# trvon/yams

Measured on AMD Instinct MI355X. Metric: k-NN QPS + recall@k, 100M x 768 fp32 cosine top-100; ingest GB/s SHA-256+CDC, higher is better.
Workload: dtype i8 (MFMA filter, exact i32 accumulate) + f64 (exact re-score)

## Files before the change

yams_amd/csrc/scan_api.cpp:

```cpp
#include <chrono>
#include <algorithm>
#include <cmath>
#include <cstdio>
#include <cstdlib>
#include <cstring>
#include <vector>

#include "accel_ctx.h"
#include "scan_launch.h"

using namespace yams_accel;

namespace {

constexpr uint64_t kMfmaMinRows = 4096;
constexpr uint64_t kExactKeyBudget = 1ull << 31;
constexpr size_t kStatWords = 16;

uint32_t round_up(uint32_t v, uint32_t m) { return (v + m - 1) / m * m; }

ScanPlan make_plan(uint64_t n_rows, uint32_t dim, uint32_t nq, uint32_t k, bool bf16, int passes, bool l2_band, int depth = 0) {
    ScanPlan p;
    p.n_rows = n_rows; p.dim = dim; p.n_queries = nq;
    p.tile_rows = bf16 ? 256 : kTileRows;
// ... 460 lines not shown
    const uint32_t nq = b.nq; const bool i8 = f.i8, bf16 = f.bf16;
    ScanLaunch& L = f.L; const ScanPlan& plan = L.plan;
    if (i8) L.dense = nullptr;
    else YA_TRY(ws_get(ctx, "dense", static_cast<size_t>(nq) * plan.sample_rows * 4, (void**)&L.dense));
    YA_TRY(ws_get(ctx, "gmax", static_cast<size_t>(nq) * plan.n_groups * 4, (void**)&L.gmax));
    YA_TRY(ws_get(ctx, "tau", static_cast<size_t>(nq) * 4, (void**)&f.d_tau));
    YA_TRY(ws_get(ctx, "list", static_cast<size_t>(nq) * plan.list_cap * 8, (void**)&f.d_list));
    const uint32_t gchunks = (plan.n_groups + kSelectCap - 1) / kSelectCap;
    YA_TRY(ws_get(ctx, "work32", static_cast<size_t>(2) * nq * std::max(1u, gchunks) * plan.tau_rank * 4, (void**)&f.d_work32));
    const uint32_t lchunks = (plan.list_cap + kSelectCap - 1) / kSelectCap, keep_max = kRescoreMax + 1;
    YA_TRY(ws_get(ctx, "work64", static_cast<size_t>(2) * nq * lchunks * keep_max * 8, (void**)&f.d_work64));
    L.tau = f.d_tau; L.tau_out = f.d_tau; L.list_count = b.d_lcount; L.list = f.d_list;
    if (i8) {
        L.i8_q_form = i8_takes_q_form(L, f.bf16_version);
        if (corpus->row_mask && corpus->row_mask_count) L.i8_mask_inflation = static_cast<double>(corpus->n_rows) / static_cast<double>(corpus->row_mask_count);
        const uint64_t regions = i8_log_regions(L);
        L.log_cap = i8_log_capacity(L);
        YA_TRY(ws_get(ctx, "i8_log_key", static_cast<size_t>(regions) * L.log_cap * i8_log_entry_bytes(L), (void**)&L.log_key));
        YA_TRY(ws_get(ctx, "i8_log_q", static_cast<size_t>(regions) * L.log_cap * 4, (void**)&L.log_q));
        const uint64_t sync_words = i8_sync_words(L);
        const size_t z_cnt = (static_cast<size_t>(regions) * 4 + 255) & ~size_t(255), z_over = (static_cast<size_t>(nq) * 4 + 255) & ~size_t(255);
        unsigned char* zeroed;
        YA_TRY(ws_get(ctx, "i8_zeroed", z_cnt + z_over + static_cast<size_t>(sync_words) * 4, (void**)&zeroed));
        YA_HIP(ctx, launch_prep_i8(st, b.d_qprep, nq, L.q_pad, b.dim, const_cast<int8_t*>(L.q_i8), const_cast<float*>(L.q_meta), L.i8_l2,
                                   reinterpret_cast<uint32_t*>(zeroed), (z_cnt + z_over) / 4 + sync_words, (corpus->i8_flags & YAMS_SCAN_I8_ROTATED) != 0));
        L.log_cnt = reinterpret_cast<uint32_t*>(zeroed);
        L.q_over = f.d_qover = reinterpret_cast<uint32_t*>(zeroed + z_cnt);
        if (sync_words) L.i8_sync = reinterpret_cast<uint32_t*>(zeroed + z_cnt + z_over);
    }
    { TimedRegion tr(ctx, "scan_sample");
      if (i8) YA_HIP(ctx, launch_scan_i8(st, L, 0, f.bf16_version));
      else if (bf16) YA_HIP(ctx, launch_scan_bf16(st, L, b.metric, 0, f.passes, f.bf16_version)); else YA_HIP(ctx, launch_scan_sample(st, L, b.metric));
      tr.end(); }
    if (b.retry) YA_HIP(ctx, hipMemcpyAsync(f.d_tau, b.retry->forced_tau, static_cast<size_t>(nq) * 4, hipMemcpyDeviceToDevice, st));
    else YA_HIP(ctx, launch_select_tau(st, L, f.d_work32));
    if (i8 && L.i8_l2) {
        YA_HIP(ctx, launch_i8_l2_thresholds(st, f.d_tau, L.q_meta, nq, L.q_pad, b.dim, b.d_l2_stats, const_cast<float*>(L.q_thr), const_cast<uint32_t*>(L.i8_q_bias)));
        YA_HIP(ctx, launch_i8_l2_rows(st, corpus->rows_nsq, corpus->rows_i8_meta, b.d_l2_nmin, corpus->n_rows, b.d_l2_stats, const_cast<float*>(L.i8_l2_meta),
                                      const_cast<uint8_t*>(L.i8_row_bias)));
    } else if (i8) YA_HIP(ctx, launch_i8_thresholds(st, f.d_tau, L.q_meta, nq, L.q_pad, const_cast<float*>(L.q_thr)));
    if (i8) YA_HIP(ctx, launch_i8_collect_sample(st, L)); else YA_HIP(ctx, launch_collect_sample(st, L));
    if (i8 && L.i8_l2) YA_HIP(ctx, launch_i8_l2_add_special(st, L, b.d_l2_special, b.l2_n_special));
    { GatedSweep gs(ctx, st);
      TimedRegion tr(ctx, "scan_filter");
      if (i8) YA_HIP(ctx, launch_scan_i8(st, L, 1, f.bf16_version));
      else if (bf16) YA_HIP(ctx, launch_scan_bf16(st, L, b.metric, 1, f.passes, f.bf16_version)); else YA_HIP(ctx, launch_scan_filter(st, L, b.metric));
      tr.end();
      gs.leave(); }
    if (i8) YA_HIP(ctx, launch_i8_log_gather(st, L));
#ifdef YAMS_ACCEL_MEASURE
    if (i8 && L.i8_sync) if (const char* dump = std::getenv("YAMS_ACCEL_DUMP_SYNC")) {
        std::vector<uint32_t> h(i8_sync_words(L));
        YA_HIP(ctx, hipMemcpyAsync(h.data(), L.i8_sync, h.size() * 4, hipMemcpyDeviceToHost, st));
        YA_HIP(ctx, hipStreamSynchronize(st));
        if (FILE* fp = std::fopen(dump, "wb")) { std::fwrite(h.data(), 4, h.size(), fp); std::fclose(fp); }
    }
    const int bv = f.bf16_version;
    if (bv != 2 && bv != 3 && bv != 4 && bv != 20 && bv != 30 && bv != 40 && bv != 50 && bv != 70 && bv != 80 && !(bv >= 81 && bv <= 99)) {
        YA_HIP(ctx, hipStreamSynchronize(st));
        YA_HIP(ctx, hipMemsetAsync(b.io.out_counts, 0, static_cast<size_t>(nq) * 4, st));
        *done = true;
    }
#endif
    return YAMS_OK;
}

yams_status_t rescore(const Batch& b, const Filter& f, uint32_t n_slots, const uint32_t* d_qmap, uint32_t n_cand) {
    const yams_scan_corpus_t* corpus = b.io.corpus;
    const uint64_t* res; uint64_t res_stride;
    YA_HIP(b.ctx, launch_select_lists(b.st, f.d_list, b.d_lcount, f.L.plan.list_cap, n_slots, d_qmap, n_cand + 1, f.d_work64, &res, &res_stride));
    RescoreLaunch R{};
    R.rows = corpus->rows; R.n_rows = corpus->n_rows; R.dim = b.dim; R.queries = b.io.queries; R.qnorm = b.d_qnorm; R.tie_rank = corpus->tie_rank;
    R.rank_row = nullptr; R.row_base = corpus->row_base; R.stripe_rows = corpus->stripe_rows; R.n_stripes = corpus->n_stripes;
    R.stripe_index = corpus->stripe_index; R.cand = res; R.cand_stride = res_stride; R.n_cand = n_cand; R.tau = f.d_tau; R.list_count = b.d_lcount;
// ... 431 lines not shown
```

yams_amd/csrc/scan_i8_kernel.hip:

```cpp
#include <cstdlib>
#include <type_traits>

#include "lds_dma.h"
#include "scan_args.h"

namespace yams_accel {

using i32x4v = __attribute__((ext_vector_type(4))) int;

constexpr int I8_ROWS = 256, I8_QUERIES = 256, I8_THREADS = 512;
constexpr int I8_SLAB = 64;
constexpr int I8_NST = 4;
constexpr int I8_A_BYTES = I8_ROWS * I8_SLAB;
constexpr int I8_B_BYTES = I8_QUERIES * I8_SLAB;
constexpr int I8_STAGE = I8_A_BYTES + I8_B_BYTES;
constexpr int I8_BLOCK_ROWS = 64;

__device__ __forceinline__ int i8_swz(int row) {
    const int j = (row >> 2) & 3;
    return (((j ^ (j >> 1)) & 1) << 1) | (j >> 1);
}

__host__ __device__ __forceinline__ uint64_t i8_blocked_offset(uint64_t row, uint32_t col, uint32_t dim) {
    const uint32_t j = static_cast<uint32_t>(row & 15u), slab = col >> 6, chunk = (col >> 4) & 3u;
    const uint32_t g = (j >> 2) & 3u, swz = (((g ^ (g >> 1)) & 1u) << 1) | (g >> 1);
    return ((row >> 4) * (dim >> 6) + slab) * 1024u + j * 64u + ((chunk ^ swz) << 4) + (col & 15u);
}

__device__ __forceinline__ int i8_neg_threshold(float A, float is, float B, float g) {
    const float t = fmaf(-A, is, fmaf(B, g, 2.0f));
    return static_cast<int>(__builtin_amdgcn_fmed3f(t, -1.0737418e9f, 1.0737418e9f));
}

__device__ __forceinline__ float i8_l2_bound(float u, float nsq, float eps) {
    const float t1 = sqrtf(nsq) * u;
    return fmaf(eps, fmaf(0.5f, nsq, fabsf(t1)), fmaf(-0.5f, nsq, t1));
}
// ... 875 lines not shown
    const uint32_t n = log_cnt[r];
    if (n == 0) return;
    const uint32_t q0 = ((r >> 3) % n_qt) * R_QUERIES;
    const int tid = threadIdx.x;
    if (tid < R_QUERIES) hist[tid] = 0u;
    __syncthreads();
    const uint64_t* keys = log_key + static_cast<uint64_t>(r) * log_cap;
    const uint32_t* qs = log_q + static_cast<uint64_t>(r) * log_cap;
    for (uint32_t i = tid; i < n; i += 256) {
        const uint32_t q = qs[i];
        uint32_t row; float u;
        if (!L2 || i8_entry_score<L2>(keys[i], q, rows_meta, q_meta, q_thr, l2, row, u)) atomicAdd(&hist[q - q0], 1u);
    }
    __syncthreads();
    if (tid < R_QUERIES) {
        const uint32_t c = hist[tid];
        slot0[tid] = c ? atomicAdd(&list_count[q0 + tid], c) : 0u;
        hist[tid] = 0u;
    }
    __syncthreads();
    for (uint32_t i = tid; i < n; i += 256) {
        const uint32_t q = qs[i];
        uint32_t row; float u;
        if (!i8_entry_score<L2>(keys[i], q, rows_meta, q_meta, q_thr, l2, row, u)) continue;
        const uint32_t pos = slot0[q - q0] + atomicAdd(&hist[q - q0], 1u);
        if (pos < list_cap) list[static_cast<uint64_t>(q) * list_cap + pos] = pack_key(u, row);
    }
}

#ifdef YAMS_ACCEL_MEASURE
#include "scan_i8q_gather.h"
#endif

__global__ __launch_bounds__(256) void i8_collect_sample_kernel(const uint32_t* gmax, uint32_t n_groups, uint32_t n_queries,
                                                                const int8_t* rows_i8, const float* rows_meta, const int8_t* q_i8,
                                                                const float* q_meta, uint32_t q_pad, uint32_t dim,
                                                                uint32_t stride, uint64_t n_rows, const uint32_t* row_mask,
                                                                const float* tau, uint32_t* list_count, uint64_t* list,
                                                                uint32_t list_cap, const float* l2_rows_nsq, float l2_eps) {
    const uint32_t q = blockIdx.y;
    const float t = tau[q];
    const uint32_t* gm = gmax + static_cast<uint64_t>(q) * n_groups;
    const uint32_t nchunk = dim / 16;
    const int lane = threadIdx.x & 63;
    const float4 qm = reinterpret_cast<const float4*>(q_meta)[q];
    const uint32_t wave0 = (blockIdx.x * blockDim.x + threadIdx.x) & ~63u, wstep = gridDim.x * blockDim.x;
    for (uint32_t g0 = wave0; g0 < n_groups; g0 += wstep) {
        const uint32_t gl = g0 + static_cast<uint32_t>(lane);
        const bool hot = gl < n_groups && !(ord2f(gm[gl]) < t);
        for (uint64_t hm = __builtin_amdgcn_ballot_w64(hot); hm; hm &= hm - 1) {
            const uint32_t g = g0 + static_cast<uint32_t>(__builtin_ctzll(hm));
            const int i = lane & 15;
            const uint64_t sidx = static_cast<uint64_t>(g >> 2) * 64 + 4 * (g & 3) + 16 * (i >> 2) + (i & 3);
            const uint64_t row = (sidx / I8_ROWS) * stride * I8_ROWS + (sidx % I8_ROWS);
            const bool ok = row < n_rows && (!row_mask || row_allowed(row_mask, row));
            const uint64_t rr = row < n_rows ? row : n_rows - 1;
            int dot = 0;
            for (uint32_t ch = static_cast<uint32_t>(lane >> 4); ch < nchunk; ch += 4) {
                const int4 xv = *reinterpret_cast<const int4*>(rows_i8 + i8_blocked_offset(rr, ch * 16, dim));
                const int4 qv = *reinterpret_cast<const int4*>(q_i8 + (static_cast<uint64_t>(ch >> 2) * q_pad + q) * 64 + (ch & 3u) * 16);
                dot = __builtin_amdgcn_sdot4(xv.x, qv.x, dot, false);
                dot = __builtin_amdgcn_sdot4(xv.y, qv.y, dot, false);
                dot = __builtin_amdgcn_sdot4(xv.z, qv.z, dot, false);
                dot = __builtin_amdgcn_sdot4(xv.w, qv.w, dot, false);
            }
            dot += __shfl_xor(dot, 16);
            dot += __shfl_xor(dot, 32);
            if (lane < 16 && ok) {
                const float2 bm = reinterpret_cast<const float2*>(rows_meta)[row / I8_BLOCK_ROWS];
                const float S = bm.x * qm.x, K = fmaf(bm.y, qm.y, qm.z);
                float u = fmaf(static_cast<float>(dot), S, K);
                bool unbounded = false;
                if (l2_rows_nsq) {
                    const float nsq = l2_rows_nsq[row];
                    unbounded = !norm_in_range(nsq);
                    u = i8_l2_bound(u, nsq, l2_eps);
                }
                if (!unbounded && !(u < t)) {
                    const uint32_t pos = atomicAdd(&list_count[q], 1u);
                    if (pos < list_cap) list[static_cast<uint64_t>(q) * list_cap + pos] = pack_key(u, static_cast<uint32_t>(row));
                }
            }
        }
    }
}

__device__ inline uint32_t rot_sign(uint32_t i, uint32_t salt) {
    uint32_t v = i * 2654435761u + salt * 0x9E3779B9u;
    v ^= v >> 15; v *= 2246822519u; v ^= v >> 13; v *= 3266489917u; v ^= v >> 16;
    return v << 31;
}
__device__ inline void wave_lds_fence() {
    __builtin_amdgcn_fence(__ATOMIC_ACQ_REL, "wavefront");
    __builtin_amdgcn_wave_barrier();
}
template <int EPL>
__device__ inline void wave_fwht(float* w, int lane, uint32_t g0, uint32_t sign_salt, float scale) {
    float v[EPL];
#pragma unroll
    for (int i = 0; i < EPL; ++i) {
        const uint32_t idx = static_cast<uint32_t>(lane) * EPL + i;
        float x = w[idx];
        if (sign_salt) x = __uint_as_float(__float_as_uint(x) ^ rot_sign(g0 + idx, sign_salt));
        v[i] = x;
    }
#pragma unroll
    for (int len = 1; len < EPL; len <<= 1)
#pragma unroll
        for (int i = 0; i < EPL; ++i)
            if (!(i & len)) { const float a = v[i], b = v[i + len]; v[i] = a + b; v[i + len] = a - b; }
#pragma unroll
    for (int m = 1; m < 64; m <<= 1)
#pragma unroll
        for (int i = 0; i < EPL; ++i) {
            const float o = __shfl_xor(v[i], m);
            v[i] = (lane & m) ? o - v[i] : v[i] + o;
// ... 527 lines not shown
#ifdef YAMS_ACCEL_MEASURE
bool i8_takes_q_form(const ScanLaunch& L, int version) {
    if (L.i8_l2 || L.plan.dim % (64u * Q_DEPTH) != 0 || L.plan.dim < 128u * Q_DEPTH) return false;
    if (!i8_resident_plan(L).use) return false;
    return version >= 70 && version <= 72;
}
uint32_t i8_log_entry_bytes(const ScanLaunch& L) { return L.i8_q_form ? Q_BLK_DWORDS * 4u : 8u; }
#else
bool i8_takes_q_form(const ScanLaunch&, int) { return false; }
uint32_t i8_log_entry_bytes(const ScanLaunch&) { return 8u; }
#endif

uint64_t i8_log_regions(const ScanLaunch& L) {
    const ResidentPlan r = i8_resident_plan(L);
    if (r.use && L.i8_q_form) return static_cast<uint64_t>(r.n_streams) * r.n_qt * 4u;
    if (r.use) return static_cast<uint64_t>(r.n_streams) * r.n_qt * 8u;
    return static_cast<uint64_t>((2u * L.plan.n_filter_tiles + 7) / 8) * L.plan.n_qtiles * 8u * 4u;
}

hipError_t launch_i8_collect_sample(hipStream_t st, const ScanLaunch& L) {
    if (L.plan.sample_rows == 0 || L.plan.n_groups == 0) return hipSuccess;
    uint32_t gx = (L.plan.n_groups + 255) / 256;
    if (gx > 64) gx = 64;
#ifdef YAMS_ACCEL_MEASURE
    if (const char* e = std::getenv("YAMS_ACCEL_COLLECT_GX")) { const uint32_t v = static_cast<uint32_t>(std::atoi(e)); if (v >= 1 && v < gx) gx = v; }
#endif
    hipLaunchKernelGGL(i8_collect_sample_kernel, dim3(gx, L.plan.n_queries), dim3(256), 0, st, L.gmax, L.plan.n_groups,
                       L.plan.n_queries, L.rows_i8, L.rows_i8_meta, L.q_i8, L.q_meta, L.q_pad, L.plan.dim, L.plan.sample_stride,
                       L.plan.n_rows, L.row_mask, L.tau, L.list_count, L.list, L.plan.list_cap,
                       L.i8_l2 ? L.rows_nsq : nullptr, L.l2_eps);
    return hipGetLastError();
}

uint64_t i8_sync_words(const ScanLaunch& L) {
    const ResidentPlan r = i8_resident_plan(L);
    return r.use ? static_cast<uint64_t>(r.n_streams) * 12u * 32u * 2u : 0u;
}

uint32_t i8_log_capacity(const ScanLaunch& L) {
    const ScanPlan& p = L.plan;
    const ResidentPlan r = i8_resident_plan(L);
    if (r.use && L.i8_q_form) {
        const double total = static_cast<double>(p.n_queries) * p.tau_rank * p.sample_stride * (L.i8_mask_inflation < 8.0 ? L.i8_mask_inflation : 8.0);
        const double share = total / (static_cast<double>(r.n_streams) * r.n_qt * 4.0);
        const double cap = 4.0 * share + 512.0;
        const uint64_t c = static_cast<uint64_t>(cap < 1.0e6 ? cap : 1.0e6);
        return static_cast<uint32_t>((c + 15) / 16 * 16);
    }
    if (r.use) {
        const double total = static_cast<double>(p.n_queries) * p.tau_rank * p.sample_stride;
        const double share = total / (static_cast<double>(r.n_streams) * r.n_qt * 8.0);
        const double cap = (L.i8_l2 ? 8.0 : 4.0) * share + 256.0;
        const uint64_t c = static_cast<uint64_t>(cap < 4.0e6 ? cap : 4.0e6);
        return static_cast<uint32_t>((c + 15) / 16 * 16);
    }
    const double per_wave = 8192.0 * p.tau_rank * p.sample_stride / static_cast<double>(p.n_rows ? p.n_rows : 1) * (L.i8_l2 ? 2.0 : 1.0);
    const uint32_t c = static_cast<uint32_t>(per_wave * 4.0 < 8192.0 ? per_wave * 4.0 : 8192.0) + 16;
    return (c + 15) / 16 * 16 < 8192u ? (c + 15) / 16 * 16 : 8192u;
}

hipError_t launch_i8_log_gather(hipStream_t st, const ScanLaunch& L) {
    const uint64_t regions = i8_log_regions(L);
    if (regions == 0) return hipSuccess;
    const ResidentPlan rp = i8_resident_plan(L);
    const I8GatherL2 l2{L.i8_l2_meta, L.i8_row_bias, L.i8_q_bias, L.rows_nsq, L.tau, L.l2_eps};
#ifdef YAMS_ACCEL_MEASURE
// ... 144 lines not shown
```

yams_amd/csrc/scan_kernels.hip:

```cpp
#include <algorithm>

#include "common.h"
#include "scan_args.h"

namespace yams_accel {

using f32x16 = __attribute__((ext_vector_type(16))) float;

constexpr int LDP = kSlabK + 4;
constexpr int STAGE_FLOATS = (kTileRows + kTileQueries) * LDP;
constexpr int SCAN_THREADS = 256;


template <int MODE, int METRIC>
__global__ __launch_bounds__(SCAN_THREADS, 2) void scan_tiles_kernel(ScanArgs a) {
    __shared__ __attribute__((aligned(16))) float lds[2 * STAGE_FLOATS];

    const uint32_t bid = blockIdx.x;
    const uint32_t xcd = bid & 7u;
    const uint32_t w = bid >> 3;
    const uint32_t qt = w % a.n_qtiles;
    const uint32_t sel = (w / a.n_qtiles) * 8u + xcd;
    if (sel >= a.n_sel_tiles) return;
    uint32_t tile;
    if (MODE == MODE_SAMPLE) tile = sel * a.stride;
    else tile = sel + sel / (a.stride - 1u) + 1u;

    const int tid = threadIdx.x;
    const int lane = tid & 63;
    const int wid = tid >> 6;
    const int wr = wid >> 1, wq = wid & 1;
    const int h = lane >> 5, l31 = lane & 31;

    const uint64_t row0 = static_cast<uint64_t>(tile) * kTileRows;
    const uint32_t q0 = qt * kTileQueries;
    const uint32_t dim = a.dim;
// ... 357 lines not shown
        if (e < keep) dst[e] = v[i];
    }
    for (uint32_t i = 256u * E + t; i < keep; i += 256) dst[i] = K(0);
}

template <typename K, int CAP>
__global__ __launch_bounds__(256) void topk_block_kernel(const K* in, const uint32_t* in_counts,
                                                         uint64_t in_stride, uint32_t n_fixed,
                                                         uint32_t count_clip, K* out,
                                                         uint64_t out_stride, uint32_t keep,
                                                         const uint32_t* qmap) {
    static_assert(CAP == 4096, "the register forms below cover 256 .. 4096 keys");
    __shared__ K s[CAP];
    const uint32_t qslot = blockIdx.y;
    const uint32_t q = qmap ? qmap[qslot] : qslot;
    uint32_t n = in_counts ? in_counts[q] : n_fixed;
    if (n > count_clip) n = count_clip;
    const uint64_t c0 = static_cast<uint64_t>(blockIdx.x) * CAP;
    const K* src = in + static_cast<uint64_t>(q) * in_stride;
    K* dst = out + static_cast<uint64_t>(qslot) * out_stride + static_cast<uint64_t>(blockIdx.x) * keep;
    if (c0 >= n) {
        for (uint32_t i = threadIdx.x; i < keep; i += 256) dst[i] = K(0);
        return;
    }
    const uint64_t left = n - c0;
    const uint64_t end = left < static_cast<uint64_t>(CAP) ? n : c0 + CAP;
    if (left <= 256) topk_block_sorted<K, 1>(src, c0, end, dst, keep, s);
    else if (left <= 512) topk_block_sorted<K, 2>(src, c0, end, dst, keep, s);
    else if (left <= 1024) topk_block_sorted<K, 4>(src, c0, end, dst, keep, s);
    else if (left <= 2048) topk_block_sorted<K, 8>(src, c0, end, dst, keep, s);
    else topk_block_sorted<K, 16>(src, c0, end, dst, keep, s);
}

constexpr int TAU_LIST = 2048;
__global__ __launch_bounds__(256) void tau_select_kernel(const uint32_t* gmax, uint32_t n_groups,
                                                         uint32_t rank, float* tau, const float* rows_meta, uint64_t n_blocks,
                                                         const float* q_meta, uint32_t rank2, uint32_t max_groups, float e_scale) {
    __shared__ uint32_t hist[2048];
    __shared__ uint32_t s_prefix, s_rank, s_count, s_v1, s_v2, s_va;
    __shared__ float s_red[4];
    const uint32_t q = blockIdx.x;
    const uint32_t* keys = gmax + static_cast<uint64_t>(q) * n_groups;
    if (n_groups < rank) {
        if (threadIdx.x == 0) tau[q] = -__builtin_inff();
        return;
    }
    if (rank >= 1 && rank <= 256) {
        const float e_mine = rows_meta != nullptr && n_blocks ? rows_meta[2 * ((n_blocks - 1) * threadIdx.x / 255) + 1] : 0.f;
        uint32_t mine = 0;
        for (uint32_t i = threadIdx.x; i < n_groups; i += 256) { const uint32_t k = keys[i]; mine = k > mine ? k : mine; }
        hist[threadIdx.x] = mine;
        if (threadIdx.x == 0) { s_count = 0; s_v1 = 0; s_v2 = 0; s_va = 0; }
        __syncthreads();
        uint32_t above = 0, at_or_above = 0;
        for (int j = 0; j < 256; ++j) { const uint32_t o = hist[j]; above += o > mine; at_or_above += o >= mine; }
        if (above < rank && rank <= at_or_above) s_prefix = mine;
        __syncthreads();
        const uint32_t L = s_prefix;
        __syncthreads();
        bool overflow = false;
        if (mine >= L)
            for (uint32_t i = threadIdx.x; i < n_groups; i += 256) {
                const uint32_t k = keys[i];
                if (k >= L) {
                    const uint32_t pos = atomicAdd(&s_count, 1u);
                    if (pos < TAU_LIST) hist[pos] = k; else overflow = true;
                }
            }
        if (!__syncthreads_or(overflow)) {
            const uint32_t c = s_count;
            if (max_groups > n_groups / 64) max_groups = n_groups / 64;
            const bool aware = rows_meta != nullptr && rank2 >= 5 && rank2 < rank && max_groups >= rank2;
            const uint32_t rank_a = rank2 - 4;
            for (uint32_t i = threadIdx.x; i < c; i += 256) {
                const uint32_t k = hist[i];
                uint32_t gt = 0, ge = 0;
                for (uint32_t j = 0; j < c; ++j) { const uint32_t o = hist[j]; gt += o > k; ge += o >= k; }
                if (gt < rank && rank <= ge) {
                    if (aware) s_v1 = k; else tau[q] = k ? ord2f(k) : -__builtin_inff();
                }
                if (aware && gt < rank2 && rank2 <= ge) s_v2 = k;
                if (aware && gt < rank_a && rank_a <= ge) s_va = k;
            }
            if (!aware) return;
            float e = e_mine;
#pragma unroll
            for (int d = 32; d >= 1; d >>= 1) e = fmaxf(e, __shfl_xor(e, d));
            if ((threadIdx.x & 63) == 0) s_red[threadIdx.x >> 6] = e;
            __syncthreads();
            const uint32_t v1 = s_v1, v2 = s_v2, va = s_va;
            float t_out = v1 ? ord2f(v1) : -__builtin_inff();
            bool want = false;
            float tp = 0.f;
            if (v1 && v2 && va) {
                e = fmaxf(fmaxf(s_red[0], s_red[1]), fmaxf(s_red[2], s_red[3]));
                const float4 qm = reinterpret_cast<const float4*>(q_meta)[q];
                const float E = fmaf(e, qm.y, qm.z) * e_scale;
                tp = ord2f(v2) - 2.0f * E;
                want = ord2f(va) - t_out < E && tp < t_out;
            }
            if (want) {
                const uint32_t lb = __syncthreads_count(mine != 0 && !(ord2f(mine) < tp));
                uint32_t n_reach = 0xffffffffu;
                if (lb <= max_groups) {
                    uint32_t cnt = 0;
                    for (uint32_t i = threadIdx.x; i < n_groups; i += 256) { const uint32_t k = keys[i]; cnt += k != 0 && !(ord2f(k) < tp); }
#pragma unroll
                    for (int d = 32; d >= 1; d >>= 1) cnt += __shfl_xor(cnt, d);
                    __syncthreads();
                    if ((threadIdx.x & 63) == 0) s_red[threadIdx.x >> 6] = __uint_as_float(cnt);
                    __syncthreads();
                    n_reach = __float_as_uint(s_red[0]) + __float_as_uint(s_red[1]) + __float_as_uint(s_red[2]) + __float_as_uint(s_red[3]);
                }
                if (n_reach <= max_groups) t_out = tp;
            }
            if (threadIdx.x == 0) tau[q] = t_out;
            return;
        }
        __syncthreads();
    }
    if (threadIdx.x == 0) { s_prefix = 0; s_rank = rank; }
    const int shifts[3] = {21, 10, 0};
    const int widths[3] = {11, 11, 10};
    for (int p = 0; p < 3; ++p) {
        const int shift = shifts[p], bins = 1 << widths[p];
        for (int i = threadIdx.x; i < 2048; i += 256) hist[i] = 0;
        __syncthreads();
        const uint32_t prefix = s_prefix;
        const int hi_shift = shift + widths[p];
        for (uint32_t i = threadIdx.x; i < n_groups; i += 256) {
            const uint32_t k = keys[i];
            if (hi_shift >= 32 || (k >> hi_shift) == prefix) atomicAdd(&hist[(k >> shift) & (bins - 1)], 1u);
        }
        __syncthreads();
        if (threadIdx.x < 64) {
            const int lane = threadIdx.x;
            const int per = bins / 64;
            uint32_t mine = 0;
            for (int j = 0; j < per; ++j) mine += hist[bins - 1 - (lane * per + j)];
            uint32_t incl = mine;
#pragma unroll
            for (int d = 1; d < 64; d <<= 1) {
                const uint32_t o = __shfl_up(incl, d);
                if (lane >= d) incl += o;
            }
            const uint32_t excl = incl - mine;
            const uint32_t r = s_rank;
            if (r > excl && r <= incl) {
                uint32_t above = excl;
                for (int j = 0; j < per; ++j) {
                    const int b = bins - 1 - (lane * per + j);
                    const uint32_t c = hist[b];
                    if (r <= above + c) { s_prefix = (prefix << widths[p]) | static_cast<uint32_t>(b); s_rank = r - above; break; }
                    above += c;
                }
            }
        }
        __syncthreads();
    }
    if (threadIdx.x == 0) {
        const uint32_t key = s_prefix;
        tau[q] = key ? ord2f(key) : -__builtin_inff();
    }
}

__global__ __launch_bounds__(256) void collect_sample_kernel(const float* dense, const uint32_t* gmax,
                                                             uint32_t n_groups, uint32_t n_queries,
                                                             uint64_t sample_rows, uint32_t tile_rows,
                                                             uint32_t stride,
                                                             uint64_t n_rows, const float* tau,
                                                             uint32_t* list_count, uint64_t* list,
                                                             uint32_t list_cap, int layout16) {
    const uint32_t q = blockIdx.y;
    const float t = tau[q];
    const uint32_t* gm = gmax + static_cast<uint64_t>(q) * n_groups;
    for (uint32_t g = blockIdx.x * blockDim.x + threadIdx.x; g < n_groups; g += gridDim.x * blockDim.x) {
        const float m = ord2f(gm[g]);
        if (m < t) continue;
        const uint64_t s0 = layout16 ? static_cast<uint64_t>(g >> 2) * 64 + 4 * (g & 3) : static_cast<uint64_t>(g >> 1) * 32 + 4 * (g & 1);
        const uint32_t gstep = layout16 ? 16u : 8u;
#pragma unroll
        for (int g4 = 0; g4 < 4; ++g4) {
            const float4 v4 = *reinterpret_cast<const float4*>(dense + dense_index(q, s0 + gstep * g4, n_queries));
            const float vv[4] = {v4.x, v4.y, v4.z, v4.w};
#pragma unroll
            for (int e = 0; e < 4; ++e) {
                const float v = vv[e];
                if (!(v < t)) {
                    const uint64_t sidx = s0 + gstep * g4 + e;
                    const uint64_t row = (sidx / tile_rows) * stride * tile_rows + (sidx % tile_rows);
                    if (row < n_rows) {
                        const uint32_t pos = atomicAdd(&list_count[q], 1u);
                        if (pos < list_cap)
                            list[static_cast<uint64_t>(q) * list_cap + pos] = pack_key(v, static_cast<uint32_t>(row));
                    }
                }
// ... 1024 lines not shown
```

yams_amd/csrc/scan_launch.h:

```cpp
#pragma once
#include "common.h"

namespace yams_accel {

struct ScanLaunch {
    ScanPlan plan;
    const float* rows = nullptr;
    const uint16_t* rows_bf16 = nullptr;
    const float* rows_nsq = nullptr;
    const int8_t* rows_i8 = nullptr;
    const float* rows_i8_meta = nullptr;
    const int8_t* q_i8 = nullptr;
    const float* q_meta = nullptr;
    const float* q_thr = nullptr;
    uint64_t* log_key = nullptr; uint32_t* log_q = nullptr; uint32_t* log_cnt = nullptr; uint32_t log_cap = 0;
    uint32_t* q_over = nullptr;
    uint32_t* i8_sync = nullptr;
    bool i8_l2 = false;
    const float* i8_l2_meta = nullptr;
    const uint8_t* i8_row_bias = nullptr;
    const uint32_t* i8_q_bias = nullptr;
    float l2_eps = 0.f;
    bool i8_sample_small_grid = false;
    int i8_form = 0;
// ... 61 lines not shown
                               int metric, float* qprep, double* qnorm, float* qnorm_up,
                               uint32_t* qflags, uint32_t* zero_words = nullptr, uint32_t n_zero_words = 0);
hipError_t launch_prep_split(hipStream_t st, const float* qprep, uint32_t nq, uint32_t q_pad, uint32_t dim,
                             uint32_t slab_k, uint16_t* q_hi, uint16_t* q_lo);
inline uint32_t bf16_slab_k(int passes, uint32_t dim) { return (passes == 1 && (dim & 31u) == 0) ? 32u : 16u; }
hipError_t launch_scan_bf16(hipStream_t st, const ScanLaunch& L, int metric, int mode, int passes, int version);
hipError_t launch_scan_i8(hipStream_t st, const ScanLaunch& L, int mode, int version);
hipError_t launch_prep_i8(hipStream_t st, const float* qprep, uint32_t nq, uint32_t q_pad, uint32_t dim,
                          int8_t* q_i8, float* q_meta, bool raw_queries = false, uint32_t* zero_words = nullptr,
                          uint64_t n_zero_words = 0, bool rotated = false);
hipError_t launch_i8_l2_norm_stats(hipStream_t st, const float* rows_nsq, const float* rows_i8_meta, uint64_t n_rows,
                                   float* nmin, uint32_t* stats, uint32_t* special);
uint32_t i8_l2_max_special();
hipError_t launch_i8_l2_add_special(hipStream_t st, const ScanLaunch& L, const uint32_t* special, uint32_t n_special);
hipError_t launch_i8_l2_thresholds(hipStream_t st, const float* tau, const float* q_meta, uint32_t nq, uint32_t q_pad,
                                   uint32_t dim, const uint32_t* stats, float* q_thr, uint32_t* q_bias);
hipError_t launch_i8_l2_rows(hipStream_t st, const float* rows_nsq, const float* rows_i8_meta, const float* nmin,
                             uint64_t n_rows, const uint32_t* stats, float* l2_meta, uint8_t* row_bias);
float i8_l2_eps(uint32_t dim);
hipError_t launch_shadow_build_i8(hipStream_t st, const float* rows, uint64_t first_row, uint64_t n_rows, uint32_t dim,
                                  int8_t* out_i8, float* out_meta, double* stats, bool rotated = false, uint64_t block_stride = 1,
                                  double* dry = nullptr);
uint32_t i8_rotation_window(uint32_t dim);
uint64_t i8_log_regions(const ScanLaunch& L);
uint32_t i8_log_capacity(const ScanLaunch& L);
bool i8_takes_resident_form(const ScanLaunch& L);
bool i8_takes_q_form(const ScanLaunch& L, int version);
uint32_t i8_log_entry_bytes(const ScanLaunch& L);
uint64_t i8_sync_words(const ScanLaunch& L);
hipError_t launch_i8_log_gather(hipStream_t st, const ScanLaunch& L);
hipError_t launch_i8_collect_sample(hipStream_t st, const ScanLaunch& L);
hipError_t launch_i8_thresholds(hipStream_t st, const float* tau, const float* q_meta, uint32_t nq, uint32_t q_pad,
                                float* q_thr);
hipError_t launch_scan_sample(hipStream_t st, const ScanLaunch& L, int metric);
hipError_t launch_scan_filter(hipStream_t st, const ScanLaunch& L, int metric);
hipError_t launch_select_tau(hipStream_t st, const ScanLaunch& L, uint32_t* work32);
hipError_t launch_collect_sample(hipStream_t st, const ScanLaunch& L);
hipError_t launch_select_lists(hipStream_t st, const uint64_t* list, const uint32_t* list_count,
                               uint32_t list_cap, uint32_t n_slots, const uint32_t* qmap,
                               uint32_t keep, uint64_t* work, const uint64_t** result,
                               uint64_t* result_stride);
hipError_t launch_exact_keys(hipStream_t st, int metric, const float* rows, uint64_t n_rows,
                             uint32_t dim, const float* queries, const double* qnorm,
                             const uint32_t* tie_rank, const uint32_t* row_mask,
                             const uint32_t* rows_sel, uint64_t n_sel, const uint32_t* qmap,
                             uint32_t n_slots, float threshold, uint32_t flags, uint64_t* keys,
                             uint64_t key_stride);
hipError_t launch_compact_rows(hipStream_t st, const uint32_t* row_mask, uint64_t n_rows,
                               const yams_scan_entity_filter_t* filters, uint32_t n_filters, const yams_scan_entities_t& cols,
                               uint32_t* rows_sel, unsigned long long* counter);
inline hipError_t launch_compact_mask(hipStream_t st, const uint32_t* row_mask, uint64_t n_rows, uint32_t* rows_sel,
                                      unsigned long long* counter) {
    return launch_compact_rows(st, row_mask, n_rows, nullptr, 0, yams_scan_entities_t{nullptr, nullptr, nullptr}, rows_sel, counter);
}
hipError_t launch_topk_keys(hipStream_t st, const uint64_t* keys, uint64_t key_stride,
                            uint32_t n_per_slot, uint32_t n_slots, uint32_t keep, uint64_t* work,
                            const uint64_t** result, uint64_t* result_stride);
hipError_t launch_rescore(hipStream_t st, int metric, const RescoreLaunch& R);
hipError_t launch_merge(hipStream_t st, const MergeLaunch& M);
hipError_t launch_shadow_build(hipStream_t st, const float* rows, uint64_t n_rows, uint32_t dim,
                               uint16_t* out_bf16, float* out_nsq);
hipError_t launch_retry_tau_l2(hipStream_t st, const float* dist, const uint32_t* counts, uint32_t k, const uint32_t* fmap, uint32_t n_slots,
                               const double* qnorm, double margin, const uint32_t* gmax, uint32_t n_groups, float* tau_out, uint32_t* est_out);
hipError_t launch_retry_tau(hipStream_t st, const float* scores, const uint32_t* counts, uint32_t k, const uint32_t* fmap, uint32_t n_slots,
                            const uint32_t* gmax, uint32_t n_groups, float* tau_out, uint32_t* est_out, float slack = 0.f);
hipError_t launch_scatter_results_from(hipStream_t st, const uint32_t* src, const uint32_t* dst, uint32_t n, uint32_t k, const float* s_scores,
// ... 16 lines not shown
```

Baseline: 17060.

## Fuse i8 tau selection, threshold computation and sample collection into one kernel

Pulls the tau selection logic into a shared device function. In the default i8 non-L2, non-retry path, one block per query now computes tau, writes the query thresholds, and then collects hot sample groups itself, with each wave handling one group. This replaces three kernel launches and the global round trips of tau and thresholds between them. Hot groups are compacted in LDS segments before collection. The collect inner loop is unrolled four-wide to raise memory-level parallelism. The trade-off is that collection now runs with one block per query rather than a 2D grid, which can lower parallelism when there are many hot groups.

```diff
diff --git a/yams_amd/csrc/scan_api.cpp b/yams_amd/csrc/scan_api.cpp
--- a/yams_amd/csrc/scan_api.cpp
+++ b/yams_amd/csrc/scan_api.cpp
@@ -516,14 +516,22 @@
       if (i8) YA_HIP(ctx, launch_scan_i8(st, L, 0, f.bf16_version));
       else if (bf16) YA_HIP(ctx, launch_scan_bf16(st, L, b.metric, 0, f.passes, f.bf16_version)); else YA_HIP(ctx, launch_scan_sample(st, L, b.metric));
       tr.end(); }
-    if (b.retry) YA_HIP(ctx, hipMemcpyAsync(f.d_tau, b.retry->forced_tau, static_cast<size_t>(nq) * 4, hipMemcpyDeviceToDevice, st));
-    else YA_HIP(ctx, launch_select_tau(st, L, f.d_work32));
-    if (i8 && L.i8_l2) {
-        YA_HIP(ctx, launch_i8_l2_thresholds(st, f.d_tau, L.q_meta, nq, L.q_pad, b.dim, b.d_l2_stats, const_cast<float*>(L.q_thr), const_cast<uint32_t*>(L.i8_q_bias)));
-        YA_HIP(ctx, launch_i8_l2_rows(st, corpus->rows_nsq, corpus->rows_i8_meta, b.d_l2_nmin, corpus->n_rows, b.d_l2_stats, const_cast<float*>(L.i8_l2_meta),
-                                      const_cast<uint8_t*>(L.i8_row_bias)));
-    } else if (i8) YA_HIP(ctx, launch_i8_thresholds(st, f.d_tau, L.q_meta, nq, L.q_pad, const_cast<float*>(L.q_thr)));
-    if (i8) YA_HIP(ctx, launch_i8_collect_sample(st, L)); else YA_HIP(ctx, launch_collect_sample(st, L));
+    bool fused_front = i8 && !L.i8_l2 && !b.retry;
+#ifdef YAMS_ACCEL_MEASURE
+    if (const char* fc = std::getenv("YAMS_ACCEL_FRONT_CHAIN")) if (std::strcmp(fc, "split") == 0) fused_front = false;
+#endif
+    if (fused_front) {
+        YA_HIP(ctx, launch_i8_tau_collect(st, L));
+    } else {
+        if (b.retry) YA_HIP(ctx, hipMemcpyAsync(f.d_tau, b.retry->forced_tau, static_cast<size_t>(nq) * 4, hipMemcpyDeviceToDevice, st));
+        else YA_HIP(ctx, launch_select_tau(st, L, f.d_work32));
+        if (i8 && L.i8_l2) {
+            YA_HIP(ctx, launch_i8_l2_thresholds(st, f.d_tau, L.q_meta, nq, L.q_pad, b.dim, b.d_l2_stats, const_cast<float*>(L.q_thr), const_cast<uint32_t*>(L.i8_q_bias)));
+            YA_HIP(ctx, launch_i8_l2_rows(st, corpus->rows_nsq, corpus->rows_i8_meta, b.d_l2_nmin, corpus->n_rows, b.d_l2_stats, const_cast<float*>(L.i8_l2_meta),
+                                          const_cast<uint8_t*>(L.i8_row_bias)));
+        } else if (i8) YA_HIP(ctx, launch_i8_thresholds(st, f.d_tau, L.q_meta, nq, L.q_pad, const_cast<float*>(L.q_thr)));
+        if (i8) YA_HIP(ctx, launch_i8_collect_sample(st, L)); else YA_HIP(ctx, launch_collect_sample(st, L));
+    }
     if (i8 && L.i8_l2) YA_HIP(ctx, launch_i8_l2_add_special(st, L, b.d_l2_special, b.l2_n_special));
     { GatedSweep gs(ctx, st);
       TimedRegion tr(ctx, "scan_filter");
diff --git a/yams_amd/csrc/scan_i8_kernel.hip b/yams_amd/csrc/scan_i8_kernel.hip
--- a/yams_amd/csrc/scan_i8_kernel.hip
+++ b/yams_amd/csrc/scan_i8_kernel.hip
@@ -3,6 +3,7 @@
 
 #include "lds_dma.h"
 #include "scan_args.h"
+#include "scan_tau_select.h"
 
 namespace yams_accel {
 
@@ -944,6 +945,55 @@
 #include "scan_i8q_gather.h"
 #endif
 
+__device__ __forceinline__ void i8_collect_group(uint32_t g, int lane, uint32_t q, float t, const float4 qm, const int8_t* rows_i8,
+                                                 const float* rows_meta, const int8_t* q_i8, uint32_t q_pad, uint32_t dim,
+                                                 uint32_t stride, uint64_t n_rows, const uint32_t* row_mask, uint32_t* list_count,
+                                                 uint64_t* list, uint32_t list_cap, const float* l2_rows_nsq, float l2_eps) {
+    const uint32_t nchunk = dim / 16;
+    const int i = lane & 15;
+    const uint64_t sidx = static_cast<uint64_t>(g >> 2) * 64 + 4 * (g & 3) + 16 * (i >> 2) + (i & 3);
+    const uint64_t row = (sidx / I8_ROWS) * stride * I8_ROWS + (sidx % I8_ROWS);
+    const bool ok = row < n_rows && (!row_mask || row_allowed(row_mask, row));
+    const uint64_t rr = row < n_rows ? row : n_rows - 1;
+    int dot = 0;
+    for (uint32_t ch0 = static_cast<uint32_t>(lane >> 4); ch0 < nchunk; ch0 += 16) {
+        int4 xv[4], qv[4];
+#pragma unroll
+        for (int u = 0; u < 4; ++u) {
+            const uint32_t ch = ch0 + 4u * u;
+            xv[u] = qv[u] = make_int4(0, 0, 0, 0);
+            if (ch < nchunk) {
+                xv[u] = *reinterpret_cast<const int4*>(rows_i8 + i8_blocked_offset(rr, ch * 16, dim));
+                qv[u] = *reinterpret_cast<const int4*>(q_i8 + (static_cast<uint64_t>(ch >> 2) * q_pad + q) * 64 + (ch & 3u) * 16);
+            }
+        }
+#pragma unroll
+        for (int u = 0; u < 4; ++u) {
+            dot = __builtin_amdgcn_sdot4(xv[u].x, qv[u].x, dot, false);
+            dot = __builtin_amdgcn_sdot4(xv[u].y, qv[u].y, dot, false);
+            dot = __builtin_amdgcn_sdot4(xv[u].z, qv[u].z, dot, false);
+            dot = __builtin_amdgcn_sdot4(xv[u].w, qv[u].w, dot, false);
+        }
+    }
+    dot += __shfl_xor(dot, 16);
+    dot += __shfl_xor(dot, 32);
+    if (lane < 16 && ok) {
+        const float2 bm = reinterpret_cast<const float2*>(rows_meta)[row / I8_BLOCK_ROWS];
+        const float S = bm.x * qm.x, K = fmaf(bm.y, qm.y, qm.z);
+        float u = fmaf(static_cast<float>(dot), S, K);
+        bool unbounded = false;
+        if (l2_rows_nsq) {
+            const float nsq = l2_rows_nsq[row];
+            unbounded = !norm_in_range(nsq);
+            u = i8_l2_bound(u, nsq, l2_eps);
+        }
+        if (!unbounded && !(u < t)) {
+            const uint32_t pos = atomicAdd(&list_count[q], 1u);
+            if (pos < list_cap) list[static_cast<uint64_t>(q) * list_cap + pos] = pack_key(u, static_cast<uint32_t>(row));
+        }
+    }
+}
+
 __global__ __launch_bounds__(256) void i8_collect_sample_kernel(const uint32_t* gmax, uint32_t n_groups, uint32_t n_queries,
                                                                 const int8_t* rows_i8, const float* rows_meta, const int8_t* q_i8,
                                                                 const float* q_meta, uint32_t q_pad, uint32_t dim,
@@ -953,47 +1003,65 @@
     const uint32_t q = blockIdx.y;
     const float t = tau[q];
     const uint32_t* gm = gmax + static_cast<uint64_t>(q) * n_groups;
-    const uint32_t nchunk = dim / 16;
     const int lane = threadIdx.x & 63;
     const float4 qm = reinterpret_cast<const float4*>(q_meta)[q];
     const uint32_t wave0 = (blockIdx.x * blockDim.x + threadIdx.x) & ~63u, wstep = gridDim.x * blockDim.x;
     for (uint32_t g0 = wave0; g0 < n_groups; g0 += wstep) {
         const uint32_t gl = g0 + static_cast<uint32_t>(lane);
         const bool hot = gl < n_groups && !(ord2f(gm[gl]) < t);
-        for (uint64_t hm = __builtin_amdgcn_ballot_w64(hot); hm; hm &= hm - 1) {
-            const uint32_t g = g0 + static_cast<uint32_t>(__builtin_ctzll(hm));
-            const int i = lane & 15;
-            const uint64_t sidx = static_cast<uint64_t>(g >> 2) * 64 + 4 * (g & 3) + 16 * (i >> 2) + (i & 3);
-            const uint64_t row = (sidx / I8_ROWS) * stride * I8_ROWS + (sidx % I8_ROWS);
-            const bool ok = row < n_rows && (!row_mask || row_allowed(row_mask, row));
-            const uint64_t rr = row < n_rows ? row : n_rows - 1;
-            int dot = 0;
-            for (uint32_t ch = static_cast<uint32_t>(lane >> 4); ch < nchunk; ch += 4) {
-                const int4 xv = *reinterpret_cast<const int4*>(rows_i8 + i8_blocked_offset(rr, ch * 16, dim));
-                const int4 qv = *reinterpret_cast<const int4*>(q_i8 + (static_cast<uint64_t>(ch >> 2) * q_pad + q) * 64 + (ch & 3u) * 16);
-                dot = __builtin_amdgcn_sdot4(xv.x, qv.x, dot, false);
-                dot = __builtin_amdgcn_sdot4(xv.y, qv.y, dot, false);
-                dot = __builtin_amdgcn_sdot4(xv.z, qv.z, dot, false);
-                dot = __builtin_amdgcn_sdot4(xv.w, qv.w, dot, false);
-            }
-            dot += __shfl_xor(dot, 16);
-            dot += __shfl_xor(dot, 32);
-            if (lane < 16 && ok) {
-                const float2 bm = reinterpret_cast<const float2*>(rows_meta)[row / I8_BLOCK_ROWS];
-                const float S = bm.x * qm.x, K = fmaf(bm.y, qm.y, qm.z);
-                float u = fmaf(static_cast<float>(dot), S, K);
-                bool unbounded = false;
-                if (l2_rows_nsq) {
-                    const float nsq = l2_rows_nsq[row];
-                    unbounded = !norm_in_range(nsq);
-                    u = i8_l2_bound(u, nsq, l2_eps);
-                }
-                if (!unbounded && !(u < t)) {
-                    const uint32_t pos = atomicAdd(&list_count[q], 1u);
-                    if (pos < list_cap) list[static_cast<uint64_t>(q) * list_cap + pos] = pack_key(u, static_cast<uint32_t>(row));
-                }
-            }
-        }
+        for (uint64_t hm = __builtin_amdgcn_ballot_w64(hot); hm; hm &= hm - 1)
+            i8_collect_group(g0 + static_cast<uint32_t>(__builtin_ctzll(hm)), lane, q, t, qm, rows_i8, rows_meta, q_i8, q_pad, dim, stride,
+                             n_rows, row_mask, list_count, list, list_cap, l2_rows_nsq, l2_eps);
+    }
+}
+
+constexpr uint32_t HOT_SEG = 4096;
+__global__ __launch_bounds__(256) void i8_tau_collect_kernel(const uint32_t* gmax, uint32_t n_groups, uint32_t nq, uint32_t rank,
+                                                             const float* tau_rows_meta, uint64_t tau_n_blocks, uint32_t rank2,
+                                                             uint32_t max_groups, float e_scale, const int8_t* rows_i8,
+                                                             const float* rows_meta, const int8_t* q_i8, const float* q_meta,
+                                                             uint32_t q_pad, uint32_t dim, uint32_t stride, uint64_t n_rows,
+                                                             const uint32_t* row_mask, float* tau, float* q_thr, uint32_t* list_count,
+                                                             uint64_t* list, uint32_t list_cap, int collect) {
+    __shared__ uint32_t s_hot[HOT_SEG];
+    __shared__ uint32_t s_nhot;
+    const uint32_t q = blockIdx.x;
+    const uint32_t* gm = gmax + static_cast<uint64_t>(q) * n_groups;
+    const float t = tau_select_block(gm, n_groups, rank, q, tau_rows_meta, tau_n_blocks, q_meta, rank2, max_groups, e_scale);
+    const float4 qm = reinterpret_cast<const float4*>(q_meta)[q];
+    if (threadIdx.x == 0) {
+        tau[q] = t;
+        float A;
+        if (t != t) A = -__builtin_inff();
+        else {
+            A = (t - qm.z) / qm.x;
+            A -= fabsf(A) * 1.9073486e-6f;
+        }
+        q_thr[2 * q] = A;
+        q_thr[2 * q + 1] = (qm.y / qm.x) * (1.0f + 1.9073486e-6f);
+    }
+    if (q == nq - 1)
+        for (uint32_t p = nq + threadIdx.x; p < q_pad; p += 256) { q_thr[2 * p] = __builtin_inff(); q_thr[2 * p + 1] = 0.f; }
+    if (!collect) return;
+    const int lane = threadIdx.x & 63;
+    const uint32_t wave = threadIdx.x >> 6;
+    for (uint32_t s0 = 0; s0 < n_groups; s0 += HOT_SEG) {
+        if (threadIdx.x == 0) s_nhot = 0;
+        __syncthreads();
+        const uint32_t s1 = n_groups - s0 < HOT_SEG ? n_groups : s0 + HOT_SEG;
+        uint32_t kk[HOT_SEG / 256];
+#pragma unroll
+        for (uint32_t u = 0; u < HOT_SEG / 256; ++u) { const uint32_t g = s0 + u * 256 + threadIdx.x; kk[u] = g < s1 ? gm[g] : 0u; }
+#pragma unroll
+        for (uint32_t u = 0; u < HOT_SEG / 256; ++u) {
+            const uint32_t g = s0 + u * 256 + threadIdx.x;
+            if (g < s1 && !(ord2f(kk[u]) < t)) s_hot[atomicAdd(&s_nhot, 1u)] = g;
+        }
+        __syncthreads();
+        const uint32_t nhot = s_nhot;
+        for (uint32_t j = wave; j < nhot; j += 4)
+            i8_collect_group(static_cast<uint32_t>(__builtin_amdgcn_readfirstlane(static_cast<int>(s_hot[j]))), lane, q, t, qm, rows_i8,
+                             rows_meta, q_i8, q_pad, dim, stride, n_rows, row_mask, list_count, list, list_cap, nullptr, 0.f);
     }
 }
 
@@ -1587,6 +1655,17 @@
     return hipGetLastError();
 }
 
+hipError_t launch_i8_tau_collect(hipStream_t st, const ScanLaunch& L) {
+    const uint32_t nq = L.plan.n_queries;
+    if (nq == 0) return hipSuccess;
+    if (L.i8_l2 || L.q_pad < nq) return hipErrorInvalidValue;
+    hipLaunchKernelGGL(i8_tau_collect_kernel, dim3(nq), dim3(256), 0, st, L.gmax, L.plan.n_groups, nq, L.plan.tau_rank, L.tau_rows_meta,
+                       L.tau_n_blocks, L.tau_rank2, L.tau_max_groups, L.tau_e_scale, L.rows_i8, L.rows_i8_meta, L.q_i8, L.q_meta, L.q_pad,
+                       L.plan.dim, L.plan.sample_stride, L.plan.n_rows, L.row_mask, L.tau_out, const_cast<float*>(L.q_thr), L.list_count,
+                       L.list, L.plan.list_cap, L.plan.sample_rows != 0 && L.plan.n_groups != 0 ? 1 : 0);
+    return hipGetLastError();
+}
+
 uint64_t i8_sync_words(const ScanLaunch& L) {
     const ResidentPlan r = i8_resident_plan(L);
     return r.use ? static_cast<uint64_t>(r.n_streams) * 12u * 32u * 2u : 0u;
diff --git a/yams_amd/csrc/scan_kernels.hip b/yams_amd/csrc/scan_kernels.hip
--- a/yams_amd/csrc/scan_kernels.hip
+++ b/yams_amd/csrc/scan_kernels.hip
@@ -2,6 +2,7 @@
 
 #include "common.h"
 #include "scan_args.h"
+#include "scan_tau_select.h"
 
 namespace yams_accel {
 
@@ -425,136 +426,13 @@
     else topk_block_sorted<K, 16>(src, c0, end, dst, keep, s);
 }
 
-constexpr int TAU_LIST = 2048;
 __global__ __launch_bounds__(256) void tau_select_kernel(const uint32_t* gmax, uint32_t n_groups,
                                                          uint32_t rank, float* tau, const float* rows_meta, uint64_t n_blocks,
                                                          const float* q_meta, uint32_t rank2, uint32_t max_groups, float e_scale) {
-    __shared__ uint32_t hist[2048];
-    __shared__ uint32_t s_prefix, s_rank, s_count, s_v1, s_v2, s_va;
-    __shared__ float s_red[4];
     const uint32_t q = blockIdx.x;
-    const uint32_t* keys = gmax + static_cast<uint64_t>(q) * n_groups;
-    if (n_groups < rank) {
-        if (threadIdx.x == 0) tau[q] = -__builtin_inff();
-        return;
-    }
-    if (rank >= 1 && rank <= 256) {
-        const float e_mine = rows_meta != nullptr && n_blocks ? rows_meta[2 * ((n_blocks - 1) * threadIdx.x / 255) + 1] : 0.f;
-        uint32_t mine = 0;
-        for (uint32_t i = threadIdx.x; i < n_groups; i += 256) { const uint32_t k = keys[i]; mine = k > mine ? k : mine; }
-        hist[threadIdx.x] = mine;
-        if (threadIdx.x == 0) { s_count = 0; s_v1 = 0; s_v2 = 0; s_va = 0; }
-        __syncthreads();
-        uint32_t above = 0, at_or_above = 0;
-        for (int j = 0; j < 256; ++j) { const uint32_t o = hist[j]; above += o > mine; at_or_above += o >= mine; }
-        if (above < rank && rank <= at_or_above) s_prefix = mine;
-        __syncthreads();
-        const uint32_t L = s_prefix;
-        __syncthreads();
-        bool overflow = false;
-        if (mine >= L)
-            for (uint32_t i = threadIdx.x; i < n_groups; i += 256) {
-                const uint32_t k = keys[i];
-                if (k >= L) {
-                    const uint32_t pos = atomicAdd(&s_count, 1u);
-                    if (pos < TAU_LIST) hist[pos] = k; else overflow = true;
-                }
-            }
-        if (!__syncthreads_or(overflow)) {
-            const uint32_t c = s_count;
-            if (max_groups > n_groups / 64) max_groups = n_groups / 64;
-            const bool aware = rows_meta != nullptr && rank2 >= 5 && rank2 < rank && max_groups >= rank2;
-            const uint32_t rank_a = rank2 - 4;
-            for (uint32_t i = threadIdx.x; i < c; i += 256) {
-                const uint32_t k = hist[i];
-                uint32_t gt = 0, ge = 0;
-                for (uint32_t j = 0; j < c; ++j) { const uint32_t o = hist[j]; gt += o > k; ge += o >= k; }
-                if (gt < rank && rank <= ge) {
-                    if (aware) s_v1 = k; else tau[q] = k ? ord2f(k) : -__builtin_inff();
-                }
-                if (aware && gt < rank2 && rank2 <= ge) s_v2 = k;
-                if (aware && gt < rank_a && rank_a <= ge) s_va = k;
-            }
-            if (!aware) return;
-            float e = e_mine;
-#pragma unroll
-            for (int d = 32; d >= 1; d >>= 1) e = fmaxf(e, __shfl_xor(e, d));
-            if ((threadIdx.x & 63) == 0) s_red[threadIdx.x >> 6] = e;
-            __syncthreads();
-            const uint32_t v1 = s_v1, v2 = s_v2, va = s_va;
-            float t_out = v1 ? ord2f(v1) : -__builtin_inff();
-            bool want = false;
-            float tp = 0.f;
-            if (v1 && v2 && va) {
-                e = fmaxf(fmaxf(s_red[0], s_red[1]), fmaxf(s_red[2], s_red[3]));
-                const float4 qm = reinterpret_cast<const float4*>(q_meta)[q];
-                const float E = fmaf(e, qm.y, qm.z) * e_scale;
-                tp = ord2f(v2) - 2.0f * E;
-                want = ord2f(va) - t_out < E && tp < t_out;
-            }
-            if (want) {
-                const uint32_t lb = __syncthreads_count(mine != 0 && !(ord2f(mine) < tp));
-                uint32_t n_reach = 0xffffffffu;
-                if (lb <= max_groups) {
-                    uint32_t cnt = 0;
-                    for (uint32_t i = threadIdx.x; i < n_groups; i += 256) { const uint32_t k = keys[i]; cnt += k != 0 && !(ord2f(k) < tp); }
-#pragma unroll
-                    for (int d = 32; d >= 1; d >>= 1) cnt += __shfl_xor(cnt, d);
-                    __syncthreads();
-                    if ((threadIdx.x & 63) == 0) s_red[threadIdx.x >> 6] = __uint_as_float(cnt);
-                    __syncthreads();
-                    n_reach = __float_as_uint(s_red[0]) + __float_as_uint(s_red[1]) + __float_as_uint(s_red[2]) + __float_as_uint(s_red[3]);
-                }
-                if (n_reach <= max_groups) t_out = tp;
-            }
-            if (threadIdx.x == 0) tau[q] = t_out;
-            return;
-        }
-        __syncthreads();
-    }
-    if (threadIdx.x == 0) { s_prefix = 0; s_rank = rank; }
-    const int shifts[3] = {21, 10, 0};
-    const int widths[3] = {11, 11, 10};
-    for (int p = 0; p < 3; ++p) {
-        const int shift = shifts[p], bins = 1 << widths[p];
-        for (int i = threadIdx.x; i < 2048; i += 256) hist[i] = 0;
-        __syncthreads();
-        const uint32_t prefix = s_prefix;
-        const int hi_shift = shift + widths[p];
-        for (uint32_t i = threadIdx.x; i < n_groups; i += 256) {
-            const uint32_t k = keys[i];
-            if (hi_shift >= 32 || (k >> hi_shift) == prefix) atomicAdd(&hist[(k >> shift) & (bins - 1)], 1u);
-        }
-        __syncthreads();
-        if (threadIdx.x < 64) {
-            const int lane = threadIdx.x;
-            const int per = bins / 64;
-            uint32_t mine = 0;
-            for (int j = 0; j < per; ++j) mine += hist[bins - 1 - (lane * per + j)];
-            uint32_t incl = mine;
-#pragma unroll
-            for (int d = 1; d < 64; d <<= 1) {
-                const uint32_t o = __shfl_up(incl, d);
-                if (lane >= d) incl += o;
-            }
-            const uint32_t excl = incl - mine;
-            const uint32_t r = s_rank;
-            if (r > excl && r <= incl) {
-                uint32_t above = excl;
-                for (int j = 0; j < per; ++j) {
-                    const int b = bins - 1 - (lane * per + j);
-                    const uint32_t c = hist[b];
-                    if (r <= above + c) { s_prefix = (prefix << widths[p]) | static_cast<uint32_t>(b); s_rank = r - above; break; }
-                    above += c;
-                }
-            }
-        }
-        __syncthreads();
-    }
-    if (threadIdx.x == 0) {
-        const uint32_t key = s_prefix;
-        tau[q] = key ? ord2f(key) : -__builtin_inff();
-    }
+    const float t = tau_select_block(gmax + static_cast<uint64_t>(q) * n_groups, n_groups, rank, q, rows_meta, n_blocks, q_meta,
+                                     rank2, max_groups, e_scale);
+    if (threadIdx.x == 0) tau[q] = t;
 }
 
 __global__ __launch_bounds__(256) void collect_sample_kernel(const float* dense, const uint32_t* gmax,
diff --git a/yams_amd/csrc/scan_launch.h b/yams_amd/csrc/scan_launch.h
--- a/yams_amd/csrc/scan_launch.h
+++ b/yams_amd/csrc/scan_launch.h
@@ -117,6 +117,7 @@
 hipError_t launch_i8_collect_sample(hipStream_t st, const ScanLaunch& L);
 hipError_t launch_i8_thresholds(hipStream_t st, const float* tau, const float* q_meta, uint32_t nq, uint32_t q_pad,
                                 float* q_thr);
+hipError_t launch_i8_tau_collect(hipStream_t st, const ScanLaunch& L);
 hipError_t launch_scan_sample(hipStream_t st, const ScanLaunch& L, int metric);
 hipError_t launch_scan_filter(hipStream_t st, const ScanLaunch& L, int metric);
 hipError_t launch_select_tau(hipStream_t st, const ScanLaunch& L, uint32_t* work32);
diff --git a/yams_amd/csrc/scan_tau_select.h b/yams_amd/csrc/scan_tau_select.h
--- /dev/null
+++ b/yams_amd/csrc/scan_tau_select.h
@@ -0,0 +1,129 @@
+#pragma once
+#include "common.h"
+#include "scan_args.h"
+
+namespace yams_accel {
+
+constexpr int TAU_LIST = 2048;
+__device__ __forceinline__ float tau_select_block(const uint32_t* keys, uint32_t n_groups, uint32_t rank, uint32_t q,
+                                                  const float* rows_meta, uint64_t n_blocks, const float* q_meta,
+                                                  uint32_t rank2, uint32_t max_groups, float e_scale) {
+    __shared__ uint32_t hist[2048];
+    __shared__ uint32_t s_prefix, s_rank, s_count, s_v1, s_v2, s_va;
+    __shared__ float s_red[4];
+    if (n_groups < rank) return -__builtin_inff();
+    if (rank >= 1 && rank <= 256) {
+        const float e_mine = rows_meta != nullptr && n_blocks ? rows_meta[2 * ((n_blocks - 1) * threadIdx.x / 255) + 1] : 0.f;
+        uint32_t mine = 0;
+        for (uint32_t i = threadIdx.x; i < n_groups; i += 256) { const uint32_t k = keys[i]; mine = k > mine ? k : mine; }
+        hist[threadIdx.x] = mine;
+        if (threadIdx.x == 0) { s_count = 0; s_v1 = 0; s_v2 = 0; s_va = 0; }
+        __syncthreads();
+        uint32_t above = 0, at_or_above = 0;
+        for (int j = 0; j < 256; ++j) { const uint32_t o = hist[j]; above += o > mine; at_or_above += o >= mine; }
+        if (above < rank && rank <= at_or_above) s_prefix = mine;
+        __syncthreads();
+        const uint32_t L = s_prefix;
+        __syncthreads();
+        bool overflow = false;
+        if (mine >= L)
+            for (uint32_t i = threadIdx.x; i < n_groups; i += 256) {
+                const uint32_t k = keys[i];
+                if (k >= L) {
+                    const uint32_t pos = atomicAdd(&s_count, 1u);
+                    if (pos < TAU_LIST) hist[pos] = k; else overflow = true;
+                }
+            }
+        if (!__syncthreads_or(overflow)) {
+            const uint32_t c = s_count;
+            if (max_groups > n_groups / 64) max_groups = n_groups / 64;
+            const bool aware = rows_meta != nullptr && rank2 >= 5 && rank2 < rank && max_groups >= rank2;
+            const uint32_t rank_a = rank2 - 4;
+            for (uint32_t i = threadIdx.x; i < c; i += 256) {
+                const uint32_t k = hist[i];
+                uint32_t gt = 0, ge = 0;
+                for (uint32_t j = 0; j < c; ++j) { const uint32_t o = hist[j]; gt += o > k; ge += o >= k; }
+                if (gt < rank && rank <= ge) s_v1 = k;
+                if (aware && gt < rank2 && rank2 <= ge) s_v2 = k;
+                if (aware && gt < rank_a && rank_a <= ge) s_va = k;
+            }
+            float e = e_mine;
+#pragma unroll
+            for (int d = 32; d >= 1; d >>= 1) e = fmaxf(e, __shfl_xor(e, d));
+            if ((threadIdx.x & 63) == 0) s_red[threadIdx.x >> 6] = e;
+            __syncthreads();
+            const uint32_t v1 = s_v1, v2 = s_v2, va = s_va;
+            float t_out = v1 ? ord2f(v1) : -__builtin_inff();
+            if (!aware) return t_out;
+            bool want = false;
+            float tp = 0.f;
+            if (v1 && v2 && va) {
+                e = fmaxf(fmaxf(s_red[0], s_red[1]), fmaxf(s_red[2], s_red[3]));
+                const float4 qm = reinterpret_cast<const float4*>(q_meta)[q];
+                const float E = fmaf(e, qm.y, qm.z) * e_scale;
+                tp = ord2f(v2) - 2.0f * E;
+                want = ord2f(va) - t_out < E && tp < t_out;
+            }
+            if (want) {
+                const uint32_t lb = __syncthreads_count(mine != 0 && !(ord2f(mine) < tp));
+                uint32_t n_reach = 0xffffffffu;
+                if (lb <= max_groups) {
+                    uint32_t cnt = 0;
+                    for (uint32_t i = threadIdx.x; i < n_groups; i += 256) { const uint32_t k = keys[i]; cnt += k != 0 && !(ord2f(k) < tp); }
+#pragma unroll
+                    for (int d = 32; d >= 1; d >>= 1) cnt += __shfl_xor(cnt, d);
+                    __syncthreads();
+                    if ((threadIdx.x & 63) == 0) s_red[threadIdx.x >> 6] = __uint_as_float(cnt);
+                    __syncthreads();
+                    n_reach = __float_as_uint(s_red[0]) + __float_as_uint(s_red[1]) + __float_as_uint(s_red[2]) + __float_as_uint(s_red[3]);
+                }
+                if (n_reach <= max_groups) t_out = tp;
+            }
+            return t_out;
+        }
+        __syncthreads();
+    }
+    if (threadIdx.x == 0) { s_prefix = 0; s_rank = rank; }
+    const int shifts[3] = {21, 10, 0};
+    const int widths[3] = {11, 11, 10};
+    for (int p = 0; p < 3; ++p) {
+        const int shift = shifts[p], bins = 1 << widths[p];
+        for (int i = threadIdx.x; i < 2048; i += 256) hist[i] = 0;
+        __syncthreads();
+        const uint32_t prefix = s_prefix;
+        const int hi_shift = shift + widths[p];
+        for (uint32_t i = threadIdx.x; i < n_groups; i += 256) {
+            const uint32_t k = keys[i];
+            if (hi_shift >= 32 || (k >> hi_shift) == prefix) atomicAdd(&hist[(k >> shift) & (bins - 1)], 1u);
+        }
+        __syncthreads();
+        if (threadIdx.x < 64) {
+            const int lane = threadIdx.x;
+            const int per = bins / 64;
+            uint32_t mine = 0;
+            for (int j = 0; j < per; ++j) mine += hist[bins - 1 - (lane * per + j)];
+            uint32_t incl = mine;
+#pragma unroll
+            for (int d = 1; d < 64; d <<= 1) {
+                const uint32_t o = __shfl_up(incl, d);
+                if (lane >= d) incl += o;
+            }
+            const uint32_t excl = incl - mine;
+            const uint32_t r = s_rank;
+            if (r > excl && r <= incl) {
+                uint32_t above = excl;
+                for (int j = 0; j < per; ++j) {
+                    const int b = bins - 1 - (lane * per + j);
+                    const uint32_t c = hist[b];
+                    if (r <= above + c) { s_prefix = (prefix << widths[p]) | static_cast<uint32_t>(b); s_rank = r - above; break; }
+                    above += c;
+                }
+            }
+        }
+        __syncthreads();
+    }
+    const uint32_t key = s_prefix;
+    return key ? ord2f(key) : -__builtin_inff();
+}
+
+}
```

Measured after the change: 17100, median of 2. Within noise of the previous version (+0.2%).
